# facebookresearch/DetectAndTrack

Measured on AMD Instinct MI355X. Metric: clips/sec (8-frame 800px), higher is better.
Workload: dtype bf16; 1 GPU; 3D R-18 FPN3D keypoint R-CNN inference, 4 clip(s) of 1x3x8x768x1344 per step (= per forward) per GPU (kT=3 body+FPN, slice-center 2D heads, per clip: 1000 proposals, 100 detections -> kps_score -> decoded keypoints); mode=infer, weights=random-init (synthetic_params, seed 3), images_per_forward=4, forwards_in_flight=3, clips_in_flight=12, keyframe_dce=False, hip_graph=True, resident_input=True, parallelism=clip-sharded x1 (no data-path collective)

## Files before the change

detectandtrack_amd/csrc/c_api.hip:

```cpp
#include <stdlib.h>

#include "dat_common.h"

int dat_ensure_ws(dat_ctx* ctx, size_t bytes) {
    if (ctx->ws_bytes >= bytes) return DAT_OK;
    const size_t want = bytes + (bytes >> 2);
    void* grown = nullptr;
    if (hipMalloc(&grown, want) != hipSuccess) {
        (void)hipGetLastError();
        DAT_FAIL(ctx, DAT_ERR_ALLOC, "workspace hipMalloc(%zu) failed", want);
    }
    if (ctx->dbg_ws_poison && (hipMemset(grown, 0xFF, want) != hipSuccess || hipDeviceSynchronize() != hipSuccess)) {
        (void)hipGetLastError();
        hipFree(grown);
        DAT_FAIL(ctx, DAT_ERR_ALLOC, "workspace poison fill failed");
    }
    if (ctx->ws) ctx->ws_retired.push_back(ctx->ws);
    ctx->ws = grown;
    ctx->ws_bytes = want;
    ctx->ws_generation++;
    return DAT_OK;
}

void dat_ctx_read_env(dat_ctx* c) {
// ... 7 lines not shown
    c->dbg_pwks = env_int("DAT_CONV_PWKS", 8);
    c->dbg_temporal = env_int("DAT_CONV_TEMPORAL", 1);
    c->dbg_wgrad_direct = env_int("DAT_WGRAD_DIRECT", 1);
    c->dbg_wgrad_ks = env_int("DAT_WGRAD_KS", 0);
    c->dbg_ablate_wgrad = env_int("DAT_WGRAD_ABLATE", 0);
    c->dbg_wgrad_sub = env_int("DAT_WGRAD_SUB", 2);
    c->dbg_pw_xcd = env_int("DAT_CONV_PW_XCD", 1);
    c->dbg_wgrad_pw = env_int("DAT_WGRAD_PW", 1);
    c->dbg_kps_sep = env_int("DAT_KPS_DECODE_SEP", 1);
    c->dbg_linear = env_int("DAT_CONV_LINEAR", 1);
    c->dbg_order = env_int("DAT_CONV_ORDER", 0);
    c->dbg_persist_pct = env_int("DAT_PERSIST_PCT", 100);
    c->dbg_bt_min = env_int("DAT_CONV_BT_MIN", 390);
    c->dbg_bt = env_int("DAT_CONV_BT", 1);
    c->dbg_mfma = env_int("DAT_CONV_MFMA", 1) == 1;
    c->dbg_roi_fold = env_int("DAT_ROI_BWD_FOLD", 1);
    c->dbg_ws_poison = env_int("DAT_WS_POISON", 0);
    c->num_cu = 0;
}

extern "C" {

int dat_version(void) { return 1; }
int dat_h16_format(void) { return DAT_H16_FORMAT; }

int dat_ctx_create(dat_ctx** out, int device) {
    if (!out) return DAT_ERR_ARG;
    int ndev = 0;
    if (hipGetDeviceCount(&ndev) != hipSuccess || device < 0 || device >= ndev) return DAT_ERR_ARG;
    if (hipSetDevice(device) != hipSuccess) return DAT_ERR_ARG;
// ... 127 lines not shown
```

detectandtrack_amd/csrc/conv3d_igemm.hip:

```cpp
#include "conv_internal.h"

using namespace dat_conv;

namespace {

template <int BP, int NTAP> struct MinWaves { static constexpr int value = (NTAP > 0 && NTAP != 10 && BP == 128) ? 3 : 2; };
template <int DT, int BN, int BP, int WAVES_N, int ONE, int NTAP, int ODT, int MF = 0>
__global__ __launch_bounds__(NTHREADS, (MinWaves<BP, NTAP>::value)) void conv3d_igemm_kernel(const ConvParams p) {
    static_assert(ONE == 1, "see the comment above");
    static_assert(!MF || (DT == DAT_BF16 && ODT == DAT_BF16 && BN == 128 && NTAP == 9), "the 16x16x32 shape exists for the bf16 128-channel dense 3x3 variants");
    constexpr int ES = ElemOf<DT>::size;
    constexpr int OES = ElemOf<ODT>::size;
    constexpr int CK = Mma<DT>::CK;
    constexpr int WAVES_P = 4 / WAVES_N;
    constexpr int WN = BN / WAVES_N;
    constexpr int WP = BP / WAVES_P;
    constexpr int MT = WN / 32;
    constexpr int PT = WP / 32;
    static_assert(MT >= 1 && PT >= 1, "tile too small");
    constexpr int MTX = MF ? 2 * MT : MT, PTX = MF ? 2 * PT : PT;
    typedef std::conditional_t<MF != 0, f32x4_t, f32x16_t> acc_t;

#ifdef DAT_CONV_TRACE
    const unsigned long long tr_k0 = __builtin_amdgcn_s_memtime();
// ... 13 lines not shown
    unsigned bid = blockIdx.x;
    if (!(p.ablate & 16)) bid = xcd_block_map(bid, p.nblocks);
    int split, nb;
    unsigned tile;
    if (p.order) {
        tile = bid % p.ntiles;
        bid /= p.ntiles;
        split = bid % p.ksplit;
        nb = bid / p.ksplit;
    } else {
        split = bid % p.ksplit;
        bid /= p.ksplit;
        nb = bid % p.nblk_n;
        tile = bid / p.nblk_n;
    }
    const int fc = tile % p.otn;
    tile /= p.otn;
    const int tw_i = tile % p.tiles_w;
    tile /= p.tiles_w;
    const int th_i = tile % p.tiles_h;
    const int clip = tile / p.tiles_h;
    const int f = clip * p.otn + fc;
    const int t = p.ot0 + fc;
    const int f_in = clip * p.T + t;
    const int n0 = nb * BN;
    const int TW = 1 << p.tw_log2;
    const int oh0 = th_i << p.th_log2;
    const int ow0 = tw_i * p.tile_w;
    const int ih0 = oh0 * p.sh - p.ph;
    const int iw0 = ow0 * p.sw - p.pw;

    int rowbase[PTX];
#pragma unroll
    for (int j = 0; j < PTX; ++j) {
        const int pos = wave_p * WP + (MF ? j * 16 + (lane & 15) : j * 32 + (lane & 31));
        const int ohl = pos >> p.tw_log2, owl = pos & (TW - 1);
        rowbase[j] = ohl * p.rsh * p.PW + owl * p.rsw;
    }
    const int khalf = lane >> 5;

    acc_t acc[MTX][PTX];
#pragma unroll
    for (int i = 0; i < MTX; ++i)
#pragma unroll
        for (int j = 0; j < PTX; ++j)
#pragma unroll
            for (int r = 0; r < (MF ? 4 : 16); ++r) acc[i][j][r] = 0.f;

    int kt_lo = 0, kt_hi = p.KT - 1;
    while (kt_lo < p.KT && (t + kt_lo - p.pt) < p.in_lo) ++kt_lo;
    while (kt_hi >= 0 && (t + kt_hi - p.pt) >= p.in_hi) --kt_hi;
    const int n_kt = kt_hi - kt_lo + 1;
    const int ntap = p.KH * p.KW;
    const int ntab = p.tab_n;
    const int npatch = n_kt * p.n_cchunks;
    const int pi_lo = (npatch * split) / p.ksplit, pi_hi = (npatch * (split + 1)) / p.ksplit;
    const int total = (pi_hi - pi_lo) * ntab;

    const int npatch_items = p.PH * p.PW * 8;

    typedef const __attribute__((address_space(1))) void* gptr_t;
    typedef __attribute__((address_space(3))) void* lptr_t;
#ifndef DAT_PATCH_AUX
#define DAT_PATCH_AUX 0
#endif
#define P_DMA(SRC_, DST_) __builtin_amdgcn_global_load_lds((gptr_t)(SRC_), (lptr_t)(DST_), 16, 0, DAT_PATCH_AUX)
#define P_COMMIT() asm volatile("s_waitcnt vmcnt(0)" ::: "memory")

    const size_t wd_cc_stride = (size_t)(p.Cout_pad >> 5) * 4096;
    const char* const wd_lane = p.w + (size_t)((n0 + wave_n * WN) >> 5) * 4096 + lane * 16;
#define WD_PTR(KT_, CC_, TI_) (wd_lane + ((size_t)((KT_) * ntap + p.tab_tap[(TI_)]) * p.n_cchunks + (CC_)) * wd_cc_stride)
    if constexpr (NTAP > 0) {
      constexpr int NT = (NTAP == 10 || NTAP == 19) ? 9 : NTAP;
      constexpr bool LIN_DIL = NTAP == 19;
      if (total > 0) {
        constexpr int MAXCH = patch_pieces_per_wave(NTAP, BP);
        const int kt_hi_x = kt_lo + n_kt;
        int kshift = 0;
        if (n_kt == p.KT && (DAT_KT_ROTATE)) kshift = (p.KT - (t + kt_lo - p.pt) % p.KT) % p.KT;
        int kt = kt_lo + pi_lo / p.n_cchunks + kshift, cc = pi_lo % p.n_cchunks;
        if (kt >= kt_hi_x) kt -= n_kt;
        constexpr bool PACK16 = NTAP != 10;
        constexpr int NQ = PACK16 ? (PTX + 1) / 2 : PTX;
        unsigned qp[NT][NQ];
        if constexpr (BP == 256) {
#pragma unroll
            for (int j = 0; j < PTX; ++j) {
                int lin_y = 0, lin_x = 0;
                if (p.lin_w > 0) {
                    const int gpos = ow0 + wave_p * WP + (MF ? j * 16 + (lane & 15) : j * 32 + (lane & 31));
                    const int rem = gpos % (p.lin_h * p.lin_w);
                    lin_y = rem / p.lin_w; lin_x = rem - lin_y * p.lin_w;
                }
#pragma unroll
                for (int tp = 0; tp < NT; ++tp) {
                    int row = rowbase[j] + p.tab_rowoff[tp];
// ... 37 lines not shown
            int off = -2;
            if (c < nchunks && it < npatch_items) {
                const int row = it >> 3;
                const int slot = patch_src_slot<MF>(it);
                const int prow = p.pw_magic ? (int)__umulhi((unsigned)row, p.pw_magic) : row, pcol = row - prow * p.PW;
                const int ih = ih0 + p.tab_dy[0] + prow * p.psh, iw = iw0 + p.tab_dx[0] + pcol * p.psw;
                off = (ih >= 0 && ih < p.H && iw >= 0 && iw < p.W && row != p.lin_zero_row) ? (int)((unsigned)(ih * p.W + iw) * (unsigned)(p.Cin * ES) + (unsigned)(slot * 16)) : -1;
            }
            poff[u] = off;
        }
        const size_t tap_stride = (size_t)p.n_cchunks * wd_cc_stride;
        const char* const wd_base = p.w + (size_t)((n0 + wave_n * WN) >> 5) * 4096;
        constexpr int NKS = MF ? 2 : 4;
        const unsigned lane16 = MF ? 16u * (((unsigned)lane & 15u) + 32u * (((unsigned)lane >> 4) & 1u)) + ((unsigned)lane >> 5) * 1024u : (unsigned)lane * 16u;
#define W_OFF(I_, KS_) (MF ? ((I_) & 1) * 256 + ((I_) >> 1) * 4096 + (KS_) * 2048 : (I_) * 4096 + (KS_) * 1024)
        const char* wcur = wd_base + ((size_t)(kt * ntap) * p.n_cchunks + cc) * wd_cc_stride;
        uint4 wa[MTX][NKS];
#pragma unroll
        for (int i = 0; i < MTX; ++i)
#pragma unroll
            for (int ks = 0; ks < NKS; ++ks) wa[i][ks] = *(const uint4*)(wcur + W_OFF(i, ks) + lane16);
        const int npat = pi_hi - pi_lo;
        for (int pi = 0; pi < npat; ++pi) {
            if (!((p.ablate & 1) && pi > 0) && !(p.x3 && pi > 0 && cc % 3 == 1)) {
                __syncthreads();
                const int fin = f_in + kt - p.pt;
                const char* xbase = p.x + ((size_t)fin * p.H * p.W) * p.Cin * ES + (size_t)(p.x3 ? (cc / 3) * 2 + (cc % 3 == 2) : cc) * CK * ES;
#pragma unroll
                for (int u = 0; u < MAXCH; ++u) {
                    int po = poff[u];
                    if constexpr (MF != 0) asm volatile("" : "+v"(po));
                    if (po != -2) {
                        const char* src = po >= 0 ? xbase + (unsigned)po : p.zeros;
                        P_DMA(src, patch + (wave + 4 * u) * 1024);
                    }
                }
                P_COMMIT();
                __syncthreads();
#ifdef DAT_CONV_TRACE
                if (!tr_first) tr_first = __builtin_amdgcn_s_memtime();
#endif
            }
            int ncc = cc + 1, nkt = kt;
            if (ncc == p.n_cchunks) { ncc = 0; if (++nkt == kt_hi_x) nkt = kt_lo; }
            const char* wnextpatch = (pi + 1 < npat) ? wd_base + ((size_t)(nkt * ntap) * p.n_cchunks + ncc) * wd_cc_stride : wcur;
            __builtin_amdgcn_s_setprio(1);
            constexpr int BF = MF ? (PT >= 4 ? 2 : PT) : PT;
            constexpr int UPS = PTX / BF, NU = NKS * UPS;
            uint4 b[2][BF];
            unsigned qa[MF ? 1 : PT];
#define Q_ADDR(TP_, J_) (!PACK16 ? qp[TP_][(J_) % NQ] : ((J_) & 1) ? (qp[TP_][((J_) >> 1) % NQ] >> 16) : (qp[TP_][((J_) >> 1) % NQ] & 0xffffu))
#pragma unroll
            for (int jj = 0; jj < NQ; ++jj) asm volatile("" : "+v"(qp[0][jj]));
            if constexpr (!MF) {
#pragma unroll
                for (int j = 0; j < PT; ++j) qa[j] = Q_ADDR(0, j);
            }
#pragma unroll
            for (int j = 0; j < BF; ++j) b[0][j] = *(const uint4*)(patch + (MF ? Q_ADDR(0, j) : qa[j % (MF ? 1 : PT)]));
#pragma unroll
            for (int tp = 0; tp < NT; ++tp) {
                const char* wnext = (tp + 1 < NT) ? wcur + (size_t)(tp + 1) * tap_stride : wnextpatch;
#pragma unroll
                for (int u = 0; u < NU; ++u) {
                    const int cur = u & 1, nxt = cur ^ 1;
                    const int ks = u / UPS, jb = (u % UPS) * BF;
                    if (u + 1 < NU) {
                        const int nks = (u + 1) / UPS, njb = ((u + 1) % UPS) * BF;
#pragma unroll
                        for (int j = 0; j < BF; ++j)
                            b[nxt][j] = *(const uint4*)(patch + ((MF ? Q_ADDR(tp, njb + j) : qa[j % (MF ? 1 : PT)]) ^ (unsigned)(nks << (MF ? 6 : 5))));
                    } else if (tp + 1 < NT) {
#pragma unroll
                        for (int jj = 0; jj < NQ; ++jj) asm volatile("" : "+v"(qp[tp + 1 < NT ? tp + 1 : tp][jj]));
                        if constexpr (!MF) {
#pragma unroll
                            for (int j = 0; j < PT; ++j) qa[j] = Q_ADDR(tp + 1 < NT ? tp + 1 : tp, j);
                        }
#pragma unroll
                        for (int j = 0; j < BF; ++j) b[nxt][j] = *(const uint4*)(patch + (MF ? Q_ADDR(tp + 1 < NT ? tp + 1 : tp, j) : qa[j % (MF ? 1 : PT)]));
                    }
#pragma unroll
                    for (int i = 0; i < MTX; ++i)
#pragma unroll
                        for (int j = 0; j < BF; ++j) {
                            if constexpr (MF) acc[i][jb + j] = DAT_MFMA16K32(wa[i][ks], b[cur][j], acc[i][jb + j]);
                            else Mma<DT>::step(wa[i][ks], b[cur][j], acc[i][j]);
                        }
                    if ((u + 1) % UPS == 0) {
#pragma unroll
                        for (int i = 0; i < MTX; ++i) wa[i][ks] = *(const uint4*)(wnext + W_OFF(i, ks) + lane16);
                    }
                    __builtin_amdgcn_sched_barrier(0);
                }
            }
#undef Q_ADDR
            __builtin_amdgcn_s_setprio(0);
            wcur = wnextpatch;
            cc = ncc; kt = nkt;
        }
#ifdef DAT_CONV_TRACE
        tr_k1 = __builtin_amdgcn_s_memtime();
        tr_unrolled = 1;
#endif
      }
    } else
    if (total > 0) {
        static_assert(!MF, "the table-driven loop runs 32x32x16 only");
        const int kt_hi_x = kt_lo + n_kt;
        int kshift = 0;
        if (n_kt == p.KT && (DAT_KT_ROTATE)) kshift = (p.KT - (t + kt_lo - p.pt) % p.KT) % p.KT;
        int kt = kt_lo + pi_lo / p.n_cchunks + kshift, cc = pi_lo % p.n_cchunks, ti = 0;
        if (kt >= kt_hi_x) kt -= n_kt;
        uint4 wa[MT][4];
// ... 64 lines not shown
                    bx[j] = g >> 1;
                }
                uint4 b[2][PT];
#pragma unroll
                for (int j = 0; j < PT; ++j) b[0][j] = *(const uint4*)(bp[j] + (bx[j] << 5));
#pragma unroll
                for (int ks = 0; ks < 4; ++ks) {
                    const int cur = ks & 1, nxt = cur ^ 1;
                    if (ks < 3) {
#pragma unroll
                        for (int j = 0; j < PT; ++j) b[nxt][j] = *(const uint4*)(bp[j] + (((ks + 1) ^ bx[j]) << 5));
                    }
#pragma unroll
                    for (int i = 0; i < MT; ++i)
#pragma unroll
                        for (int j = 0; j < PT; ++j) Mma<DT>::step(wa[i][ks], b[cur][j], acc[i][j]);
#pragma unroll
                    for (int i = 0; i < MT; ++i) wa[i][ks] = *(const uint4*)(wnext + i * 4096 + ks * 1024);
                    __builtin_amdgcn_sched_barrier(0);
                }
            }
            __builtin_amdgcn_s_setprio(0);
            ti = nti; cc = ncc; kt = nkt;
            TR_ADD(tr_mma);
        }
#ifdef DAT_CONV_TRACE
        if (tid == 0 && p.dbg) {
            atomicAdd(&p.dbg[0], tr_reload); atomicAdd(&p.dbg[1], tr_wait); atomicAdd(&p.dbg[2], tr_bar);
            atomicAdd(&p.dbg[3], tr_issue); atomicAdd(&p.dbg[4], tr_mma); atomicAdd(&p.dbg[5], (unsigned long long)total);
            atomicAdd(&p.dbg[6], __builtin_amdgcn_s_memtime() - tr_c0);
            atomicAdd(&p.dbg[7], __builtin_amdgcn_s_memrealtime() - tr_r0);
// ... 13 lines not shown
    __syncthreads();
    char* est = smem + wave * (32 * EPI_PITCH);
    const int sl_c = (lane % LPP) * CPL;
    const int sl_p = lane / LPP;
    const int cbase = n0 + wave_n * WN;
    const int c_st = cbase + sl_c;
    const bool part_mode = p.ksplit > 1;
    float sc[CPL], bi[CPL];
#pragma unroll
    for (int e = 0; e < CPL; ++e) {
        const bool ok = (c_st + e) < p.Cout;
        sc[e] = (!part_mode && p.scale && ok) ? p.scale[c_st + e] : 1.f;
        bi[e] = (!part_mode && p.bias && ok) ? p.bias[c_st + e] : 0.f;
    }
    const size_t npos_all = (size_t)p.frames * p.Ho * p.Wo;
    const size_t tile_pos = ((size_t)f * p.Ho + oh0) * p.Wo + ow0;
    char* const ybase = p.y + tile_pos * p.out_cs * OES;
    const char* const rbase = p.res_mode == 2 ? p.res + (size_t)f * (p.Ho >> 1) * (p.Wo >> 1) * p.out_cs * OES
                                              : p.res + tile_pos * p.out_cs * OES;
    const char* const abase = p.res2 + tile_pos * p.out_cs * OES;
    float* const pbase = part_mode ? p.part + ((size_t)split * npos_all + tile_pos) * p.Cout : nullptr;
    constexpr int NQ = 32 / PPI;
    const bool m4 = p.res_mode == 4;
    const bool res_pre = p.res_mode && !m4 && !part_mode && (p.out_cs & 7) == 0 && c_st + CPL <= p.Cout;
    uint4 rq[2][NQ];
    auto res_fetch = [&](int j, uint4* dst) __attribute__((always_inline)) {
#pragma unroll
        for (int q = 0; q < NQ; ++q) {
            const int pos = wave_p * WP + j * 32 + q * PPI + sl_p;
            const int ohl = pos >> p.tw_log2, owl = pos & (TW - 1);
            const int oh = oh0 + ohl, ow = ow0 + owl;
            const bool live = oh < p.Ho && ow < p.Wo && !(p.ablate & 4);
            unsigned rpos = (unsigned)(ohl * p.Wo + owl);
            if (p.res_mode == 2) rpos = (unsigned)((oh >> 1) * (p.Wo >> 1) + (ow >> 1));
            dst[q] = *(const uint4*)(rbase + (live ? (rpos * (unsigned)p.out_cs + (unsigned)c_st) * (unsigned)OES : 0u));
        }
    };
    if (res_pre) res_fetch(0, rq[0]);
#pragma unroll
    for (int j = 0; j < PT; ++j) {
        if (res_pre && j + 1 < PT) res_fetch(j + 1, rq[(j + 1) & 1]);
        if constexpr (MF) {
#pragma unroll
            for (int i = 0; i < MTX; ++i)
#pragma unroll
                for (int jl = 0; jl < 2; ++jl) epi_stage16(est, lane, i, jl, acc[i][(2 * j + jl) % PTX]);
        } else {
#pragma unroll
            for (int i = 0; i < MT; ++i)
#pragma unroll
                for (int g = 0; g < 4; ++g)
                    *(float4*)(est + (lane & 31) * EPI_PITCH + (i * 32 + g * 8 + khalf * 4) * 4) =
                        make_float4(acc[i][j][g * 4 + 0], acc[i][j][g * 4 + 1], acc[i][j][g * 4 + 2], acc[i][j][g * 4 + 3]);
        }
        __builtin_amdgcn_wave_barrier();
#pragma unroll
        for (int q = 0; q < NQ; ++q) {
            const int pl = q * PPI + sl_p;
            float v[CPL];
#pragma unroll
            for (int e4 = 0; e4 < CPL / 4; ++e4) {
                const float4 t = *(const float4*)(est + pl * EPI_PITCH + (sl_c + e4 * 4) * 4);
                v[e4 * 4 + 0] = t.x; v[e4 * 4 + 1] = t.y; v[e4 * 4 + 2] = t.z; v[e4 * 4 + 3] = t.w;
            }
            const int pos = wave_p * WP + j * 32 + pl;
            const int ohl = pos >> p.tw_log2, owl = pos & (TW - 1);
            const int oh = oh0 + ohl, ow = ow0 + owl;
            if (oh >= p.Ho || ow >= p.Wo || c_st >= p.Cout || (p.ablate & 4)) continue;
// ... 70 lines not shown
#pragma unroll
                for (int e2 = 0; e2 < CPL / 2; ++e2) o[e2] = f2bf2(v[2 * e2], v[2 * e2 + 1]);
                if (nch == CPL && (p.out_cs & 7) == 0) {
                    *(uint4*)yp = make_uint4(o[0], o[1], o[2], o[3]);
                } else {
                    *(uint2*)yp = make_uint2(o[0], o[1]);
                    if (nch > 4) *(uint2*)(yp + 8) = make_uint2(o[2], o[3]);
                }
            } else {
                *(float4*)yp = make_float4(v[0], v[1], v[2], v[3]);
                if (ODT == DAT_F32 && DT == DAT_BF16 && p.y_split)
                    split_hi_lo_store(p.y_split + ((tile_pos + lpos) * (size_t)(2 * p.out_cs) + (size_t)((c_st >> 6) * 128 + (c_st & 63))) * 2, v);
            }
        }
        __builtin_amdgcn_wave_barrier();
    }
    if (p.clk && threadIdx.x == 0) {
        atomicAdd(&p.clk[0], __builtin_amdgcn_s_memtime() - clk_c0);
        atomicAdd(&p.clk[1], __builtin_amdgcn_s_memrealtime() - clk_r0);
    }
#ifdef DAT_CONV_TRACE
    const unsigned long long tr_st = __builtin_amdgcn_s_memtime();
    asm volatile("s_waitcnt vmcnt(0)" ::: "memory");
    if (tid == 0 && p.dbg) {
        const unsigned long long e = __builtin_amdgcn_s_memtime();
        atomicAdd(&p.dbg[8], e - tr_k0);
        atomicAdd(&p.dbg[9], e - tr_k1);
        if (tr_unrolled) {
            atomicAdd(&p.dbg[10], tr_first - tr_k0);
            atomicAdd(&p.dbg[11], e - tr_st);
// ... 146 lines not shown

size_t conv_patch_lds(const ConvPlan& plan) { return ((size_t)plan.patch_h * plan.patch_w * PPITCH + 1023) & ~(size_t)1023; }

struct TileCand {
    int bp;
    TileChoice tc;
    bool lin;
    long long tiles, tiles_2d;
};
TileCand tile_cand(const dat_ctx* ctx, const dat_conv_desc* d, const ConvParams& p, int dil, int bp) {
    const TileChoice tc = choose_tile(p.Ho, p.Wo, bp == 256 ? 8 : 7, p.sh, p.sw, (p.KH - 1) * dil + 1, (p.KW - 1) * dil + 1);
    const long long t2d = cdiv_ll(p.Ho, 1ll << tc.th_log2) * cdiv_ll(p.Wo, 1ll << tc.tw_log2) * p.frames;
    const long long tlin = linear_tiles(ctx, d, p, bp);
    const bool lin = tlin > 0 && tlin * 10 <= t2d * 9;
    return TileCand{bp, tc, lin, lin ? tlin : t2d, t2d};
}

struct BlockChoice {
    TileCand tile;
    int ksplit;
};
BlockChoice plan_block(const dat_ctx* ctx, const dat_conv_desc* d, const ConvParams& p, int dil, int force_ks) {
    const int force_bp = ctx->force_bp;
    const bool small_n = d->Cout <= 64;
    const int ncc = p.x3 ? d->Cin / 64 * 3 : d->Cin / (d->dtype == DAT_F32 ? 32 : 64);
    const int npatch = d->KT * ncc, npatch_min = (d->KT > 1 ? d->KT - 1 : 1) * ncc;
    const int ntaps = d->KH * d->KW;
    const long long nbn = p.Cout_pad / (small_n ? 64 : 128);
    BlockChoice pick{TileCand{0, TileChoice{0, 0}, false, 0, 0}, 1};
    double best = 1e30;
// ... 14 lines not shown
            const bool strided_taps = ntaps > 1 && (d->stride_h > 1 || d->stride_w > 1);
            const double step_us = cand_bp == 256 ? (strided_taps ? 2.8 : 2.15) : 1.35;
            const double fixed_us = 2.0 + 0.6 * ceil((double)npatch / ks);
            double t = rounds * (steps * step_us + fixed_us);
            if (ks > 1) t += 4.0 + 2.0 * ks * (double)p.frames * p.Ho * p.Wo * d->Cout * 4.0 / 3.0e6;
            if (t < best) { best = t; pick = BlockChoice{cand, ks}; }
        }
    }
    if (!pick.tile.bp) pick.tile = tile_cand(ctx, d, p, dil, 128);
    return pick;
}

int conv_plan(const dat_ctx* ctx, int num_cu, const dat_conv_desc* d, const ConvParams& p, ConvPlan* out, char (&why)[256]) {
    ConvPlan pl;
    memset(&pl, 0, sizeof(pl));
    const int dil = conv_dilation(d);
    const bool x3 = p.x3, small_n = d->Cout <= 64;
    const bool forced = ctx->force_bp || ctx->force_ks;
    const bool mask_mode = d->res_mode >= 3;
    int force_ks = ctx->force_ks;
    if (conv_plans_per_image(d) && !force_ks) {
        ConvParams p1 = p;
        if (d->frames == 1 && d->H == 1) {
            dat_conv_desc d1 = *d;
            d1.W = p1.W = d->plan_frames;
            dat_conv3d_out_shape(&d1, &p1.Ho, &p1.Wo);
        } else {
            p1.frames = d->plan_frames / d->T * p.otn;
        }
        force_ks = plan_block(ctx, d, p1, dil, 0).ksplit;
// ... 51 lines not shown
        pl.npatch_min = (d->KT > 1 ? d->KT - 1 : 1) * (x3 ? d->Cin / 64 * 3 : d->Cin / (d->dtype == DAT_F32 ? 32 : 64));
        pl.ntap = lin && dil > 1 ? 19 : ntapv;
        pl.linear = lin;
        pl.mfma = ctx->dbg_mfma && ntapv == 9 && !x3 && !small_n && d->dtype == DAT_BF16 && !(lin && dil > 1);
        pl.in_dtype = d->dtype == DAT_F32 ? DAT_F32 : DAT_BF16;
        pl.out_dtype = d->dtype == DAT_BF16 ? DAT_BF16 : DAT_F32;
        if (lin) {
            pl.th_log2 = 0; pl.tw_log2 = big ? 8 : 7;
            pl.patch_h = 1; pl.patch_w = bp + 2 * dil * (p.W + 1) + 1;
        } else {
            pl.th_log2 = bc.tile.tc.th_log2; pl.tw_log2 = bc.tile.tc.tw_log2;
            pl.patch_h = (int)(ntapv == 10 ? (th - 1) * p.sh + p.KH : th + (p.KH - 1) * dil / p.sh);
            pl.patch_w = (int)(ntapv == 10 ? (tw - 1) * p.sw + p.KW : tw + (p.KW - 1) * dil / p.sw);
        }
        blocks = (lin ? bc.tile.tiles : bc.tile.tiles_2d) * (p.Cout_pad / pl.bn) * pl.ksplit;
    }
#define DAT_PLAN_FAIL(code, ...) do { snprintf(why, sizeof(why), __VA_ARGS__); return (code); } while (0)
    if (!(blocks > 0 && blocks < (1ll << 31))) DAT_PLAN_FAIL(DAT_ERR_ARG, "conv3d: grid of %lld blocks unsupported", blocks);
    pl.blocks = (int)blocks;
    if (pl.family == DAT_CONV_GENERIC && conv_patch_lds(pl) > 160 * 1024) {
        if (dil > 1)
            DAT_PLAN_FAIL(DAT_ERR_UNSUPPORTED, "conv3d: dilation %d is unsupported for this layer: the %dx%d patch of a %dx%d tile takes %zu bytes of LDS (limit 160 KiB)",
                          dil, pl.patch_h, pl.patch_w, 1 << pl.th_log2, 1 << pl.tw_log2, conv_patch_lds(pl));
        DAT_PLAN_FAIL(DAT_ERR_ARG, "conv3d: LDS patch of %zu bytes exceeds 160 KiB (tile %dx%d, stride %dx%d)", conv_patch_lds(pl),
                      1 << pl.th_log2, 1 << pl.tw_log2, p.sh, p.sw);
    }
#undef DAT_PLAN_FAIL
    *out = pl;
    return DAT_OK;
}

template <int DT, int BN, int BP, int WAVES_N, int NTAP, int ODT, int MF = 0>
int launch_conv(dat_ctx* ctx, hipStream_t st, ConvParams& p, const ConvPlan& plan, int dil) {
    const bool linear = plan.linear;
    const int th = 1 << plan.th_log2, tw = 1 << plan.tw_log2;
    p.th_log2 = plan.th_log2; p.tw_log2 = plan.tw_log2;
    p.PH = plan.patch_h; p.PW = plan.patch_w;
    p.lin_h = p.lin_w = 0;
    p.lin_zero_row = -1;
    if (linear) {
        const bool per_frame = p.KT > 1;
        const long long total = per_frame ? (long long)p.Ho * p.Wo : (long long)p.frames * p.Ho * p.Wo;
        DAT_ENFORCE(ctx, ((NTAP == 9 && dil == 1) || (NTAP == 19 && dil > 1)) && (per_frame || p.pt == 0) && p.sh == 1 && p.sw == 1 && p.H == p.Ho && p.W == p.Wo && p.res_mode != 2 &&
                             total * std::max(p.Cin, std::max(p.out_cs, p.Cout)) * 4 < (1ll << 31),
                    "conv3d: linear tiling on an unsupported layer");
        p.lin_h = p.H; p.lin_w = p.W;
        const int wr = p.W, nr = plan.patch_w;
// ... 36 lines not shown
    p.n_cchunks = p.x3 ? p.Cin / Mma<DT>::CK / 2 * 3 : p.Cin / Mma<DT>::CK;
    p.ablate = ctx->dbg_ablate;
    p.nblk_n = p.Cout_pad / BN;
    p.ksplit = plan.ksplit;
    p.part = nullptr;
    if (p.ksplit > 1) {
        const size_t bytes = (size_t)p.ksplit * p.frames * p.Ho * p.Wo * p.Cout * sizeof(float);
        int rc = dat_ensure_ws(ctx, bytes);
        if (rc != DAT_OK) return rc;
        p.part = (float*)ctx->ws;
    }
    DAT_ENFORCE(ctx, (long long)p.Ho * p.Wo * std::max(p.out_cs, p.Cout) * 4 < (1ll << 31),
                "conv3d: one output frame of %dx%dx%d exceeds the 2-GB range of the epilogue's 32-bit offsets", p.Ho, p.Wo, p.out_cs);
    p.nblocks = (unsigned)plan.blocks;
    p.ntiles = (unsigned)(plan.blocks / (p.ksplit * p.nblk_n));
    p.order = ctx->dbg_order > 0;
    size_t lds = conv_patch_lds(plan);
    if (lds < EPI_SLICES_BYTES) lds = EPI_SLICES_BYTES;
    auto kern = conv3d_igemm_kernel<DT, BN, BP, WAVES_N, 1, NTAP, ODT, MF>;
    if (NTAP > 0) {
        DAT_ENFORCE(ctx, NTAP != 19 || linear, "conv3d: the dilated-strip variant runs linear strips only");
        DAT_ENFORCE(ctx, p.tab_n == (NTAP == 10 || NTAP == 19 ? 9 : NTAP) && p.tab_new == 1u &&
                             (((size_t)p.PH * p.PW * 8 + 63) >> 6) <= (size_t)4 * patch_pieces_per_wave(NTAP, BP) && (NTAP == 10 || (size_t)p.PH * p.PW * PPITCH < 65536),
                    "conv3d: unrolled-tap variant on an unsupported shape (%d taps, patch %dx%d)", p.tab_n, p.PH, p.PW);
        for (int i = 0; i < p.tab_n; ++i) DAT_ENFORCE(ctx, p.tab_tap[i] == i, "conv3d: unrolled-tap variant needs taps in natural order");
    }
    {
        const int rc = dat_ensure_lds(ctx, (const void*)kern, 160 * 1024);
        if (rc != DAT_OK) return rc;
    }
#ifdef DAT_CONV_TRACE
    static unsigned long long* dbg = nullptr;
    if (!dbg) hipMalloc(&dbg, 128);
    hipMemsetAsync(dbg, 0, 128, st);
// ... 74 lines not shown
    default: return big ? launch_conv<DT, BN, 256, WN, 0, ODT>(ctx, st, p, plan, dil) : launch_conv<DT, BN, 128, WN, 0, ODT>(ctx, st, p, plan, dil);
    }
}

int conv_launch(dat_ctx* ctx, hipStream_t st, ConvParams& p, const ConvPlan& plan, int dil) {
    switch (plan.family) {
    case DAT_CONV_BIGTILE: return launch_bt(ctx, st, p, plan);
    case DAT_CONV_PW256: return launch_pw256(ctx, st, p, plan);
    case DAT_CONV_PWKS: return launch_pwks(ctx, st, p, plan);
    case DAT_CONV_TKS: return launch_tks(ctx, st, p, plan);
    case DAT_CONV_PWLW: return launch_pwlw(ctx, st, p, plan);
    case DAT_CONV_WS64: return launch_ws64(ctx, st, p, plan);
    default: break;
    }
    const bool small_n = plan.bn == 64;
    if (plan.mfma)
        return plan.bp == 256 ? launch_conv<DAT_BF16, 128, 256, 2, 9, DAT_BF16, 1>(ctx, st, p, plan, dil) : launch_conv<DAT_BF16, 128, 128, 2, 9, DAT_BF16, 1>(ctx, st, p, plan, dil);
    if (plan.in_dtype == DAT_F32) return small_n ? launch_generic<DAT_F32, 64, 1, DAT_F32>(ctx, st, p, plan, dil) : launch_generic<DAT_F32, 128, 2, DAT_F32>(ctx, st, p, plan, dil);
    if (plan.out_dtype == DAT_F32)
        return small_n ? launch_generic<DAT_BF16, 64, 1, DAT_F32>(ctx, st, p, plan, dil) : launch_generic<DAT_BF16, 128, 2, DAT_F32>(ctx, st, p, plan, dil);
    return small_n ? launch_generic<DAT_BF16, 64, 1, DAT_BF16>(ctx, st, p, plan, dil) : launch_generic<DAT_BF16, 128, 2, DAT_BF16>(ctx, st, p, plan, dil);
}

}

extern "C" {

int dat_conv3d_out_shape(const dat_conv_desc* d, int* Ho, int* Wo) {
    if (!d || d->stride_h < 1 || d->stride_w < 1) return DAT_ERR_ARG;
    const int dl = dat_conv::conv_dilation(d);
// ... 88 lines not shown
```

detectandtrack_amd/csrc/conv_internal.h:

```cpp
#ifndef DAT_CONV_INTERNAL_H
#define DAT_CONV_INTERNAL_H

#include <math.h>
#include <stdlib.h>

#include <type_traits>
#include <utility>

#include "dat_common.h"

namespace dat_conv __attribute__((visibility("hidden"))) {

constexpr int PPITCH = 128;
constexpr int NTHREADS = 256;
#ifndef DAT_KT_ROTATE
#define DAT_KT_ROTATE 1
#endif

constexpr int patch_pieces_per_wave(int ntap, int bp) { return ntap == 10 ? 19 : bp >= 256 ? 14 : 10; }

struct ConvParams {
    const char* x;
    const char* w;
    const float* scale;
// ... 61 lines not shown
#include "conv_epilogue.h"

namespace dat_conv __attribute__((visibility("hidden"))) {

template <int MF>
__device__ __forceinline__ int patch_swz(int row) { return MF ? ((row >> 1) & 3) << 1 : (row >> 1) & 7; }
template <int MF>
__device__ __forceinline__ int patch_src_slot(int it) { const int row = it >> 3; return MF ? (it & 7) ^ patch_swz<1>(row) : (it ^ (row >> 1)) & 7; }
template <int MF>
__device__ __forceinline__ unsigned patch_frag_addr(int row, int kg) {
    if (MF) return (unsigned)(row * PPITCH) + (unsigned)((kg ^ patch_swz<1>(row)) << 4);
    const int g = (row >> 1) & 7;
    return (unsigned)(row * PPITCH) + (unsigned)(((kg ^ (g & 1)) << 4) | ((g >> 1) << 5));
}

template <int... I, class F>
__device__ __forceinline__ void static_for(std::integer_sequence<int, I...>, F&& f) {
    (f(std::integral_constant<int, I>{}), ...);
}


inline int cout_pad_of(const dat_conv_desc* d) {
    const int bn = d->Cout <= 64 ? 64 : 128;
    return (d->Cout + bn - 1) / bn * bn;
}

inline int conv_dilation(const dat_conv_desc* d) { return (d->KH > 1 || d->KW > 1) && d->dil_h > 1 ? d->dil_h : 1; }
inline const char* conv_dilation_refusal(const dat_conv_desc* d) {
    if (d->KH == 1 && d->KW == 1) return nullptr;
    if (d->dil_h < 0 || d->dil_w < 0) return "negative dilation";
// ... 62 lines not shown
```

detectandtrack_amd/csrc/dat_common.h:

```cpp
#pragma once
#include <hip/hip_runtime.h>
#include <stdint.h>
#include <stdio.h>
#include <string.h>

#include <string>
#include <unordered_set>
#include <vector>

#include "../../include/dat_hip.h"

struct dat_ctx {
    int device;
    std::string last_error;
    int prof_enabled;
    hipEvent_t* prof_ev;
    int prof_cap, prof_n;
    double* prof_flops;
    int* prof_tag;
    void* ws;
    size_t ws_bytes;
    std::vector<void*> ws_retired;
    int ws_generation;
    void* zeros;
// ... 9 lines not shown
    int dbg_ws64;
    int dbg_pwks;
    int dbg_pwlw;
    int dbg_wgrad_direct;
    int dbg_ablate_wgrad;
    int dbg_wgrad_sub;
    int dbg_pw_xcd;
    int dbg_wgrad_ks;
    int dbg_wgrad_pw;
    int dbg_kps_sep;
    int dbg_ws_poison;
    int dbg_roi_fold;
    int num_cu;
    int dbg_ntap;
    int dbg_mfma;
    int dbg_temporal;
    std::unordered_set<const void*> lds_attr_done;
};

static inline int dat_ensure_lds(dat_ctx* ctx, const void* kern, int bytes) {
    if (ctx->lds_attr_done.count(kern)) return DAT_OK;
    if (hipFuncSetAttribute(kern, hipFuncAttributeMaxDynamicSharedMemorySize, bytes) != hipSuccess) {
        (void)hipGetLastError();
        ctx->last_error = "hipFuncSetAttribute(MaxDynamicSharedMemorySize) failed";
        return DAT_ERR_LAUNCH;
    }
    ctx->lds_attr_done.insert(kern);
    return DAT_OK;
}

// ... 83 lines not shown
```

detectandtrack_amd/libdat.py:

```python
import ctypes as C
import os

_HERE = os.path.dirname(os.path.abspath(__file__))
H16 = os.environ.get('DAT_H16', 'bf16')
assert H16 in ('bf16', 'fp16'), 'DAT_H16: bf16 | fp16'
LIB_PATH = os.environ.get('DAT_LIB', os.path.join(_HERE, 'libdat_hip_f16.so' if H16 == 'fp16' else 'libdat_hip.so'))

DAT_F32, DAT_BF16, DAT_BF16X3 = 0, 1, 2
DAT_OK = 0


class DatError(RuntimeError):
    """Raised for a non-zero C-ABI return code; message = dat_last_error() (the CAFFE_ENFORCE analogue)."""


class ConvDesc(C.Structure):
    _fields_ = [(n, C.c_int) for n in (
        'dtype', 'frames', 'T', 'H', 'W', 'Cin', 'Cout', 'out_cstride', 'KT', 'KH', 'KW',
        'stride_h', 'stride_w', 'pad_t', 'pad_h', 'pad_w', 'relu', 'res_mode', 'out_t0', 'out_tn', 'in_t0', 'in_tn', 'plan_frames', 'dil_h', 'dil_w')]


CONV_GENERIC, CONV_BIGTILE, CONV_PW256, CONV_PWKS, CONV_TKS, CONV_PWLW, CONV_WS64 = range(7)


class ConvPlan(C.Structure):
    _fields_ = [(n, C.c_int) for n in (
        'family', 'tag', 'blocks', 'twl', 'bn', 'bp', 'ksplit', 'npatch_min', 'ntap', 'linear', 'mfma', 'th_log2', 'tw_log2',
        'patch_h', 'patch_w', 'in_dtype', 'out_dtype')]

    def as_dict(self):
        return {n: getattr(self, n) for n, _ in self._fields_}


WGRAD_REPACK, WGRAD_NINE_TAP, WGRAD_POINTWISE, WGRAD_DIRECT = range(4)


class WgradPlan(C.Structure):
    _fields_ = [(n, C.c_int) for n in (
        'family', 'variant', 'ncopies', 'npack', 'strip', 'tile_co', 'tile_ci', 'n_co_tiles', 'n_ci_tiles', 'taps', 'ksplit', 'atomic',
        'memset_first', 'finish', 'blocks', 'threads', 'lds_bytes')] + \
               [(n, C.c_longlong) for n in ('tiles', 'r_begin', 'r_end', 'nchunks')]

    def as_dict(self):
# ... 220 lines not shown
```

include/dat_hip.h:

```cpp
#ifndef DAT_HIP_H_
#define DAT_HIP_H_

#include <stddef.h>
#include <stdint.h>

#ifdef __cplusplus
extern "C" {
#endif

typedef struct dat_ctx dat_ctx;
typedef void* dat_stream;

enum { DAT_F32 = 0, DAT_BF16 = 1,
       DAT_BF16X3 = 2 };
enum { DAT_OK = 0, DAT_ERR_ARG = -1, DAT_ERR_LAUNCH = -2, DAT_ERR_ALLOC = -3, DAT_ERR_UNSUPPORTED = -4 };

int dat_version(void);
int dat_h16_format(void);
int dat_ctx_create(dat_ctx** out, int device);
void dat_ctx_destroy(dat_ctx* ctx);
const char* dat_last_error(dat_ctx* ctx);
int dat_ws_info(dat_ctx* ctx, void** ptr, size_t* bytes, int* generation);
int dat_ws_reserve(dat_ctx* ctx, size_t bytes);
int dat_fill_zero(dat_ctx* ctx, dat_stream s, void* ptr, size_t bytes);
// ... 196 lines not shown
       DAT_CONV_WS64 = 6 };
typedef struct dat_conv_plan {
    int family;
    int tag;
    int blocks;
    int twl;
    int bn, bp;
    int ksplit;
    int npatch_min;
    int ntap;
    int linear;
    int mfma;
    int th_log2, tw_log2;
    int patch_h, patch_w;
    int in_dtype, out_dtype;
} dat_conv_plan;
int dat_conv3d_plan(dat_ctx* ctx, const dat_conv_desc* d, int num_cu, dat_conv_plan* out);
int dat_conv3d_persistent_share(dat_ctx* ctx, int percent);

size_t dat_stem_conv_weight_bytes(int dtype);
int dat_stem_conv_pack_weights(dat_ctx* ctx, dat_stream s, int dtype, const float* conv1_w, int Cout, void* packed);
int dat_stem_conv(dat_ctx* ctx, dat_stream s, int dtype, const float* data, const void* w_packed, const float* scale,
                  const float* bias, int relu, int N, int T, int H, int W, void* out);

int dat_stem_conv_pool(dat_ctx* ctx, dat_stream s, int dtype, const float* data, const void* w_packed, const float* scale,
                       const float* bias, int relu, int N, int T, int H, int W, void* out_pool);
int dat_stem_conv_pool_u8(dat_ctx* ctx, dat_stream s, int dtype, const unsigned char* frames, int n_frames, int h, int w, double fx, double fy,
                          int out_h, int out_w, int pad_h, int pad_w, const double* pixel_means, const void* w_packed, const float* scale,
                          const float* bias, int relu, void* out_pool);

// ... 154 lines not shown
```

Baseline: 273.3 clips/s.

## Compute two adjacent output frames per block in stride-2 3D conv to share patches

For bf16 3x3x3 stride-2 convs with temporal pad 1, each block now computes two consecutive output frames. A schedule interleaves the temporal taps so that each loaded input patch feeds both frames' accumulators, which cuts redundant LDS patch loads and halves the grid along time. In exchange the block holds twice the accumulator registers, which may lower occupancy, and there is fewer parallelism in the grid. The path is enabled by default and can be turned off with an environment flag.

```diff
diff --git a/detectandtrack_amd/csrc/c_api.hip b/detectandtrack_amd/csrc/c_api.hip
--- a/detectandtrack_amd/csrc/c_api.hip
+++ b/detectandtrack_amd/csrc/c_api.hip
@@ -45,6 +45,7 @@
     c->dbg_bt_min = env_int("DAT_CONV_BT_MIN", 390);
     c->dbg_bt = env_int("DAT_CONV_BT", 1);
     c->dbg_mfma = env_int("DAT_CONV_MFMA", 1) == 1;
+    c->dbg_tpair = env_int("DAT_CONV_TPAIR", 1) != 0;
     c->dbg_roi_fold = env_int("DAT_ROI_BWD_FOLD", 1);
     c->dbg_ws_poison = env_int("DAT_WS_POISON", 0);
     c->num_cu = 0;
diff --git a/detectandtrack_amd/csrc/conv3d_igemm.hip b/detectandtrack_amd/csrc/conv3d_igemm.hip
--- a/detectandtrack_amd/csrc/conv3d_igemm.hip
+++ b/detectandtrack_amd/csrc/conv3d_igemm.hip
@@ -5,9 +5,10 @@
 namespace {
 
 template <int BP, int NTAP> struct MinWaves { static constexpr int value = (NTAP > 0 && NTAP != 10 && BP == 128) ? 3 : 2; };
-template <int DT, int BN, int BP, int WAVES_N, int ONE, int NTAP, int ODT, int MF = 0>
+template <int DT, int BN, int BP, int WAVES_N, int ONE, int NTAP, int ODT, int MF = 0, int TPB = 1>
 __global__ __launch_bounds__(NTHREADS, (MinWaves<BP, NTAP>::value)) void conv3d_igemm_kernel(const ConvParams p) {
     static_assert(ONE == 1, "see the comment above");
+    static_assert(TPB == 1 || (TPB == 2 && NTAP == 10 && !MF && DT == DAT_BF16 && ODT == DAT_BF16), "frame pairs exist for the 16-bit dense stride-2 variant");
     static_assert(!MF || (DT == DAT_BF16 && ODT == DAT_BF16 && BN == 128 && NTAP == 9), "the 16x16x32 shape exists for the bf16 128-channel dense 3x3 variants");
     constexpr int ES = ElemOf<DT>::size;
     constexpr int OES = ElemOf<ODT>::size;
@@ -51,8 +52,10 @@
         nb = bid % p.nblk_n;
         tile = bid / p.nblk_n;
     }
-    const int fc = tile % p.otn;
-    tile /= p.otn;
+    const int otb = TPB == 2 ? (p.otn + 1) >> 1 : p.otn;
+    const int fc = (tile % otb) * TPB;
+    tile /= otb;
+    const int nfr = TPB == 2 ? min(2, p.otn - fc) : 1;
     const int tw_i = tile % p.tiles_w;
     tile /= p.tiles_w;
     const int th_i = tile % p.tiles_h;
@@ -76,13 +79,15 @@
     }
     const int khalf = lane >> 5;
 
-    acc_t acc[MTX][PTX];
+    acc_t acc[TPB][MTX][PTX];
+#pragma unroll
+    for (int fq = 0; fq < TPB; ++fq)
 #pragma unroll
     for (int i = 0; i < MTX; ++i)
 #pragma unroll
         for (int j = 0; j < PTX; ++j)
 #pragma unroll
-            for (int r = 0; r < (MF ? 4 : 16); ++r) acc[i][j][r] = 0.f;
+            for (int r = 0; r < (MF ? 4 : 16); ++r) acc[fq][i][j][r] = 0.f;
 
     int kt_lo = 0, kt_hi = p.KT - 1;
     while (kt_lo < p.KT && (t + kt_lo - p.pt) < p.in_lo) ++kt_lo;
@@ -92,7 +97,11 @@
     const int ntab = p.tab_n;
     const int npatch = n_kt * p.n_cchunks;
     const int pi_lo = (npatch * split) / p.ksplit, pi_hi = (npatch * (split + 1)) / p.ksplit;
-    const int total = (pi_hi - pi_lo) * ntab;
+    KtRange kr1{0, 0, 0};
+    if constexpr (TPB == 2) {
+        if (nfr == 2) kr1 = kt_range(t + 1, p.KT, p.pt, p.in_lo, p.in_hi);
+    }
+    const int total = TPB == 2 ? (max(n_kt, 0) + kr1.n) * p.n_cchunks * ntab : (pi_hi - pi_lo) * ntab;
 
     const int npatch_items = p.PH * p.PW * 8;
 
@@ -117,6 +126,12 @@
         if (n_kt == p.KT && (DAT_KT_ROTATE)) kshift = (p.KT - (t + kt_lo - p.pt) % p.KT) % p.KT;
         int kt = kt_lo + pi_lo / p.n_cchunks + kshift, cc = pi_lo % p.n_cchunks;
         if (kt >= kt_hi_x) kt -= n_kt;
+        unsigned sched = 0;
+        int nsched = 0;
+        if constexpr (TPB == 2) {
+            sched = tpair_schedule(kt_range(t, p.KT, p.pt, p.in_lo, p.in_hi), kr1, &nsched);
+            kt = (int)sched & 3; cc = 0;
+        }
         constexpr bool PACK16 = NTAP != 10;
         constexpr int NQ = PACK16 ? (PTX + 1) / 2 : PTX;
         unsigned qp[NT][NQ];
@@ -184,14 +199,16 @@
         constexpr int NKS = MF ? 2 : 4;
         const unsigned lane16 = MF ? 16u * (((unsigned)lane & 15u) + 32u * (((unsigned)lane >> 4) & 1u)) + ((unsigned)lane >> 5) * 1024u : (unsigned)lane * 16u;
 #define W_OFF(I_, KS_) (MF ? ((I_) & 1) * 256 + ((I_) >> 1) * 4096 + (KS_) * 2048 : (I_) * 4096 + (KS_) * 1024)
-        const char* wcur = wd_base + ((size_t)(kt * ntap) * p.n_cchunks + cc) * wd_cc_stride;
+        const char* wcur = wd_base + ((size_t)((TPB == 2 ? tpair_first_kt(sched, 0) : kt) * ntap) * p.n_cchunks + cc) * wd_cc_stride;
         uint4 wa[MTX][NKS];
 #pragma unroll
         for (int i = 0; i < MTX; ++i)
 #pragma unroll
             for (int ks = 0; ks < NKS; ++ks) wa[i][ks] = *(const uint4*)(wcur + W_OFF(i, ks) + lane16);
-        const int npat = pi_hi - pi_lo;
+        const int npat = TPB == 2 ? nsched * p.n_cchunks : pi_hi - pi_lo;
+        int se = 0;
         for (int pi = 0; pi < npat; ++pi) {
+            const int fmask = TPB == 2 ? (int)(sched >> (4 * se + 2)) & 3 : 1;
             if (!((p.ablate & 1) && pi > 0) && !(p.x3 && pi > 0 && cc % 3 == 1)) {
                 __syncthreads();
                 const int fin = f_in + kt - p.pt;
@@ -211,9 +228,19 @@
                 if (!tr_first) tr_first = __builtin_amdgcn_s_memtime();
 #endif
             }
-            int ncc = cc + 1, nkt = kt;
-            if (ncc == p.n_cchunks) { ncc = 0; if (++nkt == kt_hi_x) nkt = kt_lo; }
-            const char* wnextpatch = (pi + 1 < npat) ? wd_base + ((size_t)(nkt * ntap) * p.n_cchunks + ncc) * wd_cc_stride : wcur;
+            int ncc = cc + 1, nkt = kt, nse = se;
+            if constexpr (TPB == 2) {
+                if (ncc == p.n_cchunks) { ncc = 0; ++nse; }
+                nkt = (int)(sched >> (4 * nse)) & 3;
+            } else {
+                if (ncc == p.n_cchunks) { ncc = 0; if (++nkt == kt_hi_x) nkt = kt_lo; }
+            }
+            const char* wnextpatch = (pi + 1 < npat) ? wd_base + ((size_t)((TPB == 2 ? tpair_first_kt(sched, nse) : nkt) * ntap) * p.n_cchunks + ncc) * wd_cc_stride : wcur;
+#pragma unroll
+            for (int fq = 0; fq < TPB; ++fq) {
+            if (TPB == 2 && !((fmask >> fq) & 1)) continue;
+            const char* wnextrun = wnextpatch;
+            if (TPB == 2 && fq == 0 && (fmask & 2)) wnextrun = wd_base + ((size_t)((kt - 1) * ntap) * p.n_cchunks + cc) * wd_cc_stride;
             __builtin_amdgcn_s_setprio(1);
             constexpr int BF = MF ? (PT >= 4 ? 2 : PT) : PT;
             constexpr int UPS = PTX / BF, NU = NKS * UPS;
@@ -230,7 +257,7 @@
             for (int j = 0; j < BF; ++j) b[0][j] = *(const uint4*)(patch + (MF ? Q_ADDR(0, j) : qa[j % (MF ? 1 : PT)]));
 #pragma unroll
             for (int tp = 0; tp < NT; ++tp) {
-                const char* wnext = (tp + 1 < NT) ? wcur + (size_t)(tp + 1) * tap_stride : wnextpatch;
+                const char* wnext = (tp + 1 < NT) ? wcur + (size_t)(tp + 1) * tap_stride : wnextrun;
 #pragma unroll
                 for (int u = 0; u < NU; ++u) {
                     const int cur = u & 1, nxt = cur ^ 1;
@@ -254,8 +281,8 @@
                     for (int i = 0; i < MTX; ++i)
 #pragma unroll
                         for (int j = 0; j < BF; ++j) {
-                            if constexpr (MF) acc[i][jb + j] = DAT_MFMA16K32(wa[i][ks], b[cur][j], acc[i][jb + j]);
-                            else Mma<DT>::step(wa[i][ks], b[cur][j], acc[i][j]);
+                            if constexpr (MF) acc[fq][i][jb + j] = DAT_MFMA16K32(wa[i][ks], b[cur][j], acc[fq][i][jb + j]);
+                            else Mma<DT>::step(wa[i][ks], b[cur][j], acc[fq][i][j]);
                         }
                     if ((u + 1) % UPS == 0) {
 #pragma unroll
@@ -266,8 +293,9 @@
             }
 #undef Q_ADDR
             __builtin_amdgcn_s_setprio(0);
-            wcur = wnextpatch;
-            cc = ncc; kt = nkt;
+            wcur = wnextrun;
+            }
+            cc = ncc; kt = nkt; se = nse;
         }
 #ifdef DAT_CONV_TRACE
         tr_k1 = __builtin_amdgcn_s_memtime();
@@ -362,7 +390,7 @@
 #pragma unroll
                     for (int i = 0; i < MT; ++i)
 #pragma unroll
-                        for (int j = 0; j < PT; ++j) Mma<DT>::step(wa[i][ks], b[cur][j], acc[i][j]);
+                        for (int j = 0; j < PT; ++j) Mma<DT>::step(wa[i][ks], b[cur][j], acc[0][i][j]);
 #pragma unroll
                     for (int i = 0; i < MT; ++i) wa[i][ks] = *(const uint4*)(wnext + i * 4096 + ks * 1024);
                     __builtin_amdgcn_sched_barrier(0);
@@ -406,9 +434,10 @@
         bi[e] = (!part_mode && p.bias && ok) ? p.bias[c_st + e] : 0.f;
     }
     const size_t npos_all = (size_t)p.frames * p.Ho * p.Wo;
-    const size_t tile_pos = ((size_t)f * p.Ho + oh0) * p.Wo + ow0;
+    for (int fq = 0;;) {
+    const size_t tile_pos = ((size_t)(f + fq) * p.Ho + oh0) * p.Wo + ow0;
     char* const ybase = p.y + tile_pos * p.out_cs * OES;
-    const char* const rbase = p.res_mode == 2 ? p.res + (size_t)f * (p.Ho >> 1) * (p.Wo >> 1) * p.out_cs * OES
+    const char* const rbase = p.res_mode == 2 ? p.res + (size_t)(f + fq) * (p.Ho >> 1) * (p.Wo >> 1) * p.out_cs * OES
                                               : p.res + tile_pos * p.out_cs * OES;
     const char* const abase = p.res2 + tile_pos * p.out_cs * OES;
     float* const pbase = part_mode ? p.part + ((size_t)split * npos_all + tile_pos) * p.Cout : nullptr;
@@ -436,14 +465,14 @@
 #pragma unroll
             for (int i = 0; i < MTX; ++i)
 #pragma unroll
-                for (int jl = 0; jl < 2; ++jl) epi_stage16(est, lane, i, jl, acc[i][(2 * j + jl) % PTX]);
+                for (int jl = 0; jl < 2; ++jl) epi_stage16(est, lane, i, jl, acc[0][i][(2 * j + jl) % PTX]);
         } else {
 #pragma unroll
             for (int i = 0; i < MT; ++i)
 #pragma unroll
                 for (int g = 0; g < 4; ++g)
                     *(float4*)(est + (lane & 31) * EPI_PITCH + (i * 32 + g * 8 + khalf * 4) * 4) =
-                        make_float4(acc[i][j][g * 4 + 0], acc[i][j][g * 4 + 1], acc[i][j][g * 4 + 2], acc[i][j][g * 4 + 3]);
+                        make_float4(acc[0][i][j][g * 4 + 0], acc[0][i][j][g * 4 + 1], acc[0][i][j][g * 4 + 2], acc[0][i][j][g * 4 + 3]);
         }
         __builtin_amdgcn_wave_barrier();
 #pragma unroll
@@ -544,6 +573,12 @@
             }
         }
         __builtin_amdgcn_wave_barrier();
+    }
+    if (TPB == 1 || ++fq >= nfr) break;
+#pragma unroll
+    for (int i = 0; i < MTX; ++i)
+#pragma unroll
+        for (int j = 0; j < PTX; ++j) acc[0][i][j] = acc[TPB - 1][i][j];
     }
     if (p.clk && threadIdx.x == 0) {
         atomicAdd(&p.clk[0], __builtin_amdgcn_s_memtime() - clk_c0);
@@ -720,6 +755,12 @@
     const long long tlin = linear_tiles(ctx, d, p, bp);
     const bool lin = tlin > 0 && tlin * 10 <= t2d * 9;
     return TileCand{bp, tc, lin, lin ? tlin : t2d, t2d};
+}
+
+bool tpair_eligible(const dat_ctx* ctx, const dat_conv_desc* d, const ConvParams& p, const ConvPlan& pl) {
+    return ctx->dbg_tpair && d->dtype == DAT_BF16 && d->KT == 3 && d->pad_t == 1 && d->KH == 3 && d->KW == 3 && d->stride_h == 2 && d->stride_w == 2 &&
+           d->pad_h == 1 && d->pad_w == 1 && conv_dilation(d) == 1 && pl.family == DAT_CONV_GENERIC && pl.ntap == 10 && pl.ksplit == 1 &&
+           pl.bn == 128 && pl.bp == 128 && d->res_mode < 3 && p.otn >= 2;
 }
 
 struct BlockChoice {
@@ -764,6 +805,7 @@
 int conv_plan(const dat_ctx* ctx, int num_cu, const dat_conv_desc* d, const ConvParams& p, ConvPlan* out, char (&why)[256]) {
     ConvPlan pl;
     memset(&pl, 0, sizeof(pl));
+    pl.frames_per_block = 1;
     const int dil = conv_dilation(d);
     const bool x3 = p.x3, small_n = d->Cout <= 64;
     const bool forced = ctx->force_bp || ctx->force_ks;
@@ -845,6 +887,7 @@
             pl.patch_w = (int)(ntapv == 10 ? (tw - 1) * p.sw + p.KW : tw + (p.KW - 1) * dil / p.sw);
         }
         blocks = (lin ? bc.tile.tiles : bc.tile.tiles_2d) * (p.Cout_pad / pl.bn) * pl.ksplit;
+        if (tpair_eligible(ctx, d, p, pl)) pl.frames_per_block = 2;
     }
 #define DAT_PLAN_FAIL(code, ...) do { snprintf(why, sizeof(why), __VA_ARGS__); return (code); } while (0)
     if (!(blocks > 0 && blocks < (1ll << 31))) DAT_PLAN_FAIL(DAT_ERR_ARG, "conv3d: grid of %lld blocks unsupported", blocks);
@@ -861,7 +904,7 @@
     return DAT_OK;
 }
 
-template <int DT, int BN, int BP, int WAVES_N, int NTAP, int ODT, int MF = 0>
+template <int DT, int BN, int BP, int WAVES_N, int NTAP, int ODT, int MF = 0, int TPB = 1>
 int launch_conv(dat_ctx* ctx, hipStream_t st, ConvParams& p, const ConvPlan& plan, int dil) {
     const bool linear = plan.linear;
     const int th = 1 << plan.th_log2, tw = 1 << plan.tw_log2;
@@ -928,10 +971,15 @@
                 "conv3d: one output frame of %dx%dx%d exceeds the 2-GB range of the epilogue's 32-bit offsets", p.Ho, p.Wo, p.out_cs);
     p.nblocks = (unsigned)plan.blocks;
     p.ntiles = (unsigned)(plan.blocks / (p.ksplit * p.nblk_n));
+    if (TPB == 2) {
+        DAT_ENFORCE(ctx, plan.frames_per_block == 2 && p.ksplit == 1 && p.otn >= 2 && p.ntiles % (unsigned)p.otn == 0, "conv3d: frame pairs on an unsupported plan");
+        p.ntiles = p.ntiles / (unsigned)p.otn * (unsigned)((p.otn + 1) / 2);
+        p.nblocks = p.ntiles * (unsigned)p.nblk_n;
+    }
     p.order = ctx->dbg_order > 0;
     size_t lds = conv_patch_lds(plan);
     if (lds < EPI_SLICES_BYTES) lds = EPI_SLICES_BYTES;
-    auto kern = conv3d_igemm_kernel<DT, BN, BP, WAVES_N, 1, NTAP, ODT, MF>;
+    auto kern = conv3d_igemm_kernel<DT, BN, BP, WAVES_N, 1, NTAP, ODT, MF, TPB>;
     if (NTAP > 0) {
         DAT_ENFORCE(ctx, NTAP != 19 || linear, "conv3d: the dilated-strip variant runs linear strips only");
         DAT_ENFORCE(ctx, p.tab_n == (NTAP == 10 || NTAP == 19 ? 9 : NTAP) && p.tab_new == 1u &&
@@ -1036,6 +1084,8 @@
     default: break;
     }
     const bool small_n = plan.bn == 64;
+    if (plan.frames_per_block == 2)
+        return launch_conv<DAT_BF16, 128, 128, 2, 10, DAT_BF16, 0, 2>(ctx, st, p, plan, dil);
     if (plan.mfma)
         return plan.bp == 256 ? launch_conv<DAT_BF16, 128, 256, 2, 9, DAT_BF16, 1>(ctx, st, p, plan, dil) : launch_conv<DAT_BF16, 128, 128, 2, 9, DAT_BF16, 1>(ctx, st, p, plan, dil);
     if (plan.in_dtype == DAT_F32) return small_n ? launch_generic<DAT_F32, 64, 1, DAT_F32>(ctx, st, p, plan, dil) : launch_generic<DAT_F32, 128, 2, DAT_F32>(ctx, st, p, plan, dil);
diff --git a/detectandtrack_amd/csrc/conv_internal.h b/detectandtrack_amd/csrc/conv_internal.h
--- a/detectandtrack_amd/csrc/conv_internal.h
+++ b/detectandtrack_amd/csrc/conv_internal.h
@@ -99,6 +99,44 @@
     return (unsigned)(row * PPITCH) + (unsigned)(((kg ^ (g & 1)) << 4) | ((g >> 1) << 5));
 }
 
+struct KtRange {
+    int lo, n, first;
+};
+__host__ __device__ inline KtRange kt_range(int t, int KT, int pt, int in_lo, int in_hi) {
+    int lo = 0, hi = KT - 1;
+    while (lo < KT && (t + lo - pt) < in_lo) ++lo;
+    while (hi >= 0 && (t + hi - pt) >= in_hi) --hi;
+    const int n = hi >= lo ? hi - lo + 1 : 0;
+    int first = lo;
+    if (n == KT && (DAT_KT_ROTATE)) first = lo + (KT - (t + lo - pt) % KT) % KT;
+    if (first >= lo + n) first -= n;
+    return KtRange{lo, n, first};
+}
+__host__ __device__ inline unsigned tpair_schedule(KtRange a, KtRange b, int* count) {
+    unsigned sched = 0, done_a = 0, done_b = 0;
+    int n = 0, ka = a.first, kb = b.first, ca = 0, cb = 0;
+    while (ca < a.n || cb < b.n) {
+        const bool ha = ca < a.n, hb = cb < b.n;
+        const int ra = ka, rb = kb + 1;
+        const bool b_needs_ra = hb && ra - 1 >= b.lo && ra - 1 < b.lo + b.n && !((done_b >> (ra - 1)) & 1u);
+        const bool a_needs_rb = ha && rb >= a.lo && rb < a.lo + a.n && !((done_a >> rb) & 1u);
+        int r = ra, m = 1;
+        if (ha && hb && ra == rb) m = 3;
+        else if (ha && !b_needs_ra) m = 1;
+        else if (hb && !a_needs_rb) { r = rb; m = 2; }
+        sched |= (unsigned)(r | (m << 2)) << (4 * n);
+        ++n;
+        if (m & 1) { done_a |= 1u << ka; ++ca; if (++ka == a.lo + a.n) ka = a.lo; }
+        if (m & 2) { done_b |= 1u << kb; ++cb; if (++kb == b.lo + b.n) kb = b.lo; }
+    }
+    *count = n;
+    return sched;
+}
+__host__ __device__ inline int tpair_first_kt(unsigned sched, int e) {
+    const int r = (sched >> (4 * e)) & 3;
+    return ((sched >> (4 * e + 2)) & 1u) ? r : r - 1;
+}
+
 template <int... I, class F>
 __device__ __forceinline__ void static_for(std::integer_sequence<int, I...>, F&& f) {
     (f(std::integral_constant<int, I>{}), ...);
diff --git a/detectandtrack_amd/csrc/dat_common.h b/detectandtrack_amd/csrc/dat_common.h
--- a/detectandtrack_amd/csrc/dat_common.h
+++ b/detectandtrack_amd/csrc/dat_common.h
@@ -47,6 +47,7 @@
     int num_cu;
     int dbg_ntap;
     int dbg_mfma;
+    int dbg_tpair;
     int dbg_temporal;
     std::unordered_set<const void*> lds_attr_done;
 };
diff --git a/detectandtrack_amd/libdat.py b/detectandtrack_amd/libdat.py
--- a/detectandtrack_amd/libdat.py
+++ b/detectandtrack_amd/libdat.py
@@ -26,7 +26,7 @@
 class ConvPlan(C.Structure):
     _fields_ = [(n, C.c_int) for n in (
         'family', 'tag', 'blocks', 'twl', 'bn', 'bp', 'ksplit', 'npatch_min', 'ntap', 'linear', 'mfma', 'th_log2', 'tw_log2',
-        'patch_h', 'patch_w', 'in_dtype', 'out_dtype')]
+        'patch_h', 'patch_w', 'in_dtype', 'out_dtype', 'frames_per_block')]
 
     def as_dict(self):
         return {n: getattr(self, n) for n, _ in self._fields_}
diff --git a/include/dat_hip.h b/include/dat_hip.h
--- a/include/dat_hip.h
+++ b/include/dat_hip.h
@@ -234,6 +234,7 @@
     int th_log2, tw_log2;
     int patch_h, patch_w;
     int in_dtype, out_dtype;
+    int frames_per_block;
 } dat_conv_plan;
 int dat_conv3d_plan(dat_ctx* ctx, const dat_conv_desc* d, int num_cu, dat_conv_plan* out);
 int dat_conv3d_persistent_share(dat_ctx* ctx, int percent);
```

After: 273.2 clips/s. No clear change (-0.1%).
